# shenyunhang/DRN-WSOD-pytorch

Hardware: AMD Instinct MI355X
Metric: images/sec training, VOC07 DRN-WSOD R50-C4 2k proposals, 1/2/4/8 GPUs (higher is better)
Workload: dtype bf16

## Files before the change

drn-wsod-pytorch_amd/csrc/gemm_conv.hip:

```cpp
#include "drn_common.h"
#include "tune.h"
#include "conv_params.h"

#include <limits.h>

namespace {

struct GemmParams {
  const char* A;
  const char* B;
  float* C;
  int M, N, K;
  long lda, ldb, ldc;
  int k_slabs_per_split;
  long c_split_stride;
  int accumulate;
  float* sgd_w;
  float* sgd_mom;
  bf16_t* sgd_shadow;
  const SgdSeg* sgd_seg;
  float sgd_momentum, sgd_grad_scale;
  int sgd_first_step;
  long sgd_ld;
  int c_bf16;
  int nsplit;
  int gm;
  int kb_rows;
  const float* sgd_acc;
  long sgd_acc_ld;
};

using drn_conv::ConvParams;

template <int DT>
__device__ __forceinline__ void mma_step(f32x16_t& acc, const i32x4_t& a, const i32x4_t& b) {
  if constexpr (DT == DRN_BF16) {
    acc = __builtin_amdgcn_mfma_f32_32x32x16_bf16(__builtin_bit_cast(bf16x8_t, a), __builtin_bit_cast(bf16x8_t, b),
                                                  acc, 0, 0, 0);
  } else if constexpr (DT == DRN_FP8) {
    typedef long i64x2_t __attribute__((ext_vector_type(2)));
    const i64x2_t al = __builtin_bit_cast(i64x2_t, a), bl = __builtin_bit_cast(i64x2_t, b);
    acc = __builtin_amdgcn_mfma_f32_32x32x16_fp8_fp8(al[0], bl[0], acc, 0, 0, 0);
    acc = __builtin_amdgcn_mfma_f32_32x32x16_fp8_fp8(al[1], bl[1], acc, 0, 0, 0);
  } else {
    const f32x4_t af = __builtin_bit_cast(f32x4_t, a), bf = __builtin_bit_cast(f32x4_t, b);
#pragma unroll
    for (int e = 0; e < 4; ++e) acc = __builtin_amdgcn_mfma_f32_32x32x2f32(af[e], bf[e], acc, 0, 0, 0);
  }
}

typedef int i32x8_t __attribute__((ext_vector_type(8)));
__device__ __forceinline__ void mma_step64_fp8(f32x16_t& acc, const i32x4_t& a0, const i32x4_t& a1, const i32x4_t& b0,
                                               const i32x4_t& b1) {
  const i32x8_t A = {a0[0], a0[1], a0[2], a0[3], a1[0], a1[1], a1[2], a1[3]};
  const i32x8_t B = {b0[0], b0[1], b0[2], b0[3], b1[0], b1[1], b1[2], b1[3]};
  acc = __builtin_amdgcn_mfma_scale_f32_32x32x64_f8f6f4(A, B, acc, 0, 0, 0, 0x7f7f7f7f, 0, 0x7f7f7f7f);
}

template <int ROWS>
__device__ __forceinline__ void lds_store_tile(char* lds, const i32x4_t (&r)[ROWS / 32], int tid) {
  const int slot = tid & 7, r0 = tid >> 3;
#pragma unroll
// ... 258 lines not shown
  float lr, wd, mom, gs;
  int first;
};
typedef float f32x2_t_ __attribute__((ext_vector_type(2)));
struct SgdRegs { f32x4_t w, m; f32x2_t_ g; };

__device__ __forceinline__ void sgdp_load(const SgdPipe& sp, SgdRegs& r, unsigned off, unsigned goff) {
  r.w = __builtin_nontemporal_load((const f32x4_t*)((const char*)sp.w + off));
  r.m = __builtin_nontemporal_load((const f32x4_t*)((const char*)sp.m + off));
  r.g = __builtin_nontemporal_load((const f32x2_t_*)((const char*)sp.g + goff));
}
__device__ __forceinline__ void sgdp_apply_store(const SgdPipe& sp, const SgdRegs& r, unsigned off) {
#pragma clang fp contract(off)
  typedef unsigned u32x2_t __attribute__((ext_vector_type(2)));
  const u32x2_t x = __builtin_bit_cast(u32x2_t, r.g);
  const f32x4_t gg = {__builtin_bit_cast(float, x.x << 16), __builtin_bit_cast(float, x.x & 0xffff0000u),
                      __builtin_bit_cast(float, x.y << 16), __builtin_bit_cast(float, x.y & 0xffff0000u)};
  f32x4_t nb, nw;
#pragma unroll
  for (int e = 0; e < 4; ++e) {
    float d = gg[e] * sp.gs;
    if (sp.wd != 0.f) d = d + sp.wd * r.w[e];
    nb[e] = sp.first ? d : sp.mom * r.m[e] + d;
    nw[e] = r.w[e] - sp.lr * nb[e];
  }
  u32x2_t o;
  o.x = (uint32_t)f32_to_bf16(nw[0]) | ((uint32_t)f32_to_bf16(nw[1]) << 16);
  o.y = (uint32_t)f32_to_bf16(nw[2]) | ((uint32_t)f32_to_bf16(nw[3]) << 16);
  __builtin_nontemporal_store(nb, (f32x4_t*)((char*)sp.m + off));
  __builtin_nontemporal_store(nw, (f32x4_t*)((char*)sp.w + off));
  *(u32x2_t*)((char*)sp.s + (off >> 1)) = o;
}

template <int DT, int VAR, bool TN = false, bool SGDP = false>
__device__ __forceinline__ void pp_mainloop(f32x16_t (&acc)[4][2], char* smem, __amdgpu_buffer_rsrc_t ra,
                                            __amdgpu_buffer_rsrc_t rb, const unsigned (&voa)[4], const unsigned (&vob)[4],
                                            int s0, int s1, int lane, int wave, unsigned bstep = 128,
                                            const SgdPipe* spp = nullptr) {
  SgdRegs srA, srB;
  const int wm = wave >> 2, wn = wave & 3;
  const int l31 = lane & 31, hi = lane >> 5, sw = (l31 >> 1) & 7;
  unsigned oa[4], ob[4];
  const unsigned lds0 = (unsigned)(uintptr_t)(__attribute__((address_space(3))) char*)smem;
#pragma unroll
  for (int ks = 0; ks < 4; ++ks) {
    oa[ks] = lds0 + PP_A0 + (wm * 64 + l31) * 128 + (((ks * 2 + hi) ^ sw) << 4);
    const int tg = lane >> 4, tj = (lane >> 2) & 3, tc = lane & 3;
    ob[ks] = TN ? lds0 + PP_B0 + (ks * 4 + 2 * (tg >> 1)) * 1024 + tj * 256 + (((wn * 2 + (tg & 1)) ^ (2 * tj)) << 5) + tc * 8
                : lds0 + PP_B0 + (wn * 32 + l31) * 128 + (((ks * 2 + hi) ^ sw) << 4);
  }
  typedef __attribute__((address_space(3))) const i32x4_t* lds_v4;
  i32x4_t fa[2][4], fb[4];
  auto rdA = [&](int ks, int off) {
    fa[0][ks] = *(lds_v4)(uintptr_t)(oa[ks] + off);
    fa[1][ks] = *(lds_v4)(uintptr_t)(oa[ks] + off + 4096);
  };
  auto rdB = [&](int ks, int off) {
    if constexpr (TN) {
      typedef int i32x2_t __attribute__((ext_vector_type(2)));
      i32x2_t l2, h2;
      const unsigned addr = ob[ks] + off;
      asm volatile("ds_read_b64_tr_b16 %0, %1" : "=v"(l2) : "v"(addr));
      asm volatile("ds_read_b64_tr_b16 %0, %1 offset:1024" : "=v"(h2) : "v"(addr));
      fb[ks] = i32x4_t{l2[0], l2[1], h2[0], h2[1]};
    } else {
      fb[ks] = *(lds_v4)(uintptr_t)(ob[ks] + off);
    }
  };
  auto mm = [&](f32x16_t& c0, f32x16_t& c1, auto wait_b_tag) {
    constexpr bool WAIT_B = decltype(wait_b_tag)::value;
    if (VAR != 3) __builtin_amdgcn_s_setprio(1);
    if constexpr (TN && WAIT_B) asm volatile("s_waitcnt lgkmcnt(6)" : "+v"(fb[0]));
    mma_step<DT>(c0, fb[0], fa[0][0]);
    mma_step<DT>(c1, fb[0], fa[1][0]);
    if constexpr (TN && WAIT_B) { __builtin_amdgcn_sched_barrier(0); asm volatile("s_waitcnt lgkmcnt(4)" : "+v"(fb[1])); }
    mma_step<DT>(c0, fb[1], fa[0][1]);
    mma_step<DT>(c1, fb[1], fa[1][1]);
    if constexpr (TN && WAIT_B) { __builtin_amdgcn_sched_barrier(0); asm volatile("s_waitcnt lgkmcnt(2)" : "+v"(fb[2])); }
    mma_step<DT>(c0, fb[2], fa[0][2]);
    mma_step<DT>(c1, fb[2], fa[1][2]);
    if constexpr (TN && WAIT_B) { __builtin_amdgcn_sched_barrier(0); asm volatile("s_waitcnt lgkmcnt(0)" : "+v"(fb[3])); }
    mma_step<DT>(c0, fb[3], fa[0][3]);
    mma_step<DT>(c1, fb[3], fa[1][3]);
    if (VAR != 3) __builtin_amdgcn_s_setprio(0);
  };
  constexpr std::false_type NOWAIT{};
  constexpr std::true_type WAITB{};
  auto piece = [&](char* stage, auto qtag, int slab) {
    constexpr int q = decltype(qtag)::value;
    constexpr int which = q >> 1, pc = q & 1;
    constexpr int off = which == 0 ? PP_A0 : which == 1 ? PP_B0 : which == 2 ? PP_B1 : PP_A1;
    constexpr bool isA = which == 0 || which == 3;
    constexpr int h = (which == 2 || which == 3) ? 1 : 0;
    char* dst = stage + off + (pc * 64 + wave * 8) * 128;
    __builtin_amdgcn_raw_ptr_buffer_load_lds(isA ? ra : rb, (__attribute__((address_space(3))) void*)dst, 16,
                                             isA ? voa[h * 2 + pc] : vob[h * 2 + pc], isA ? slab * 128 : slab * bstep, 0, 0);
  };
#define PP_PIECE(q) piece(nxt, std::integral_constant<int, q>{}, sn)
  asm volatile("s_waitcnt vmcnt(0)" ::: "memory");
  PP_BARRIER();
  if (wm == 1) PP_BARRIER();
  auto slab = [&](int s, SgdRegs& sr_ld, const SgdRegs& sr_use) __attribute__((always_inline)) {
    char* nxt = smem + (((s - s0) & 1) ^ 1) * PP_STAGE;
    const int sn = s + 1 < s1 ? s + 1 : s1 - 1;
    if constexpr (TN) {
#pragma unroll
      for (int ks = 0; ks < 4; ++ks) rdB(ks, 0);
#pragma unroll
      for (int ks = 0; ks < 4; ++ks) rdA(ks, 0);
    } else {
#pragma unroll
      for (int ks = 0; ks < 4; ++ks) { rdB(ks, 0); rdA(ks, 0); }
    }
    if (VAR == 2) {
      asm volatile("s_waitcnt vmcnt(2)" ::: "memory");
    } else {
      PP_PIECE(0); PP_PIECE(1);
      if constexpr (SGDP) {
        const unsigned i_ = (unsigned)(s - s0);
        if (i_ < 32) {
          sgdp_load(*spp, sr_ld, spp->off + i_ * spp->step, spp->goff + i_ * spp->gstep);
          asm volatile("s_waitcnt vmcnt(7)" ::: "memory");
        } else {
          asm volatile("s_waitcnt vmcnt(4)" ::: "memory");
        }
      } else {
        asm volatile("s_waitcnt vmcnt(4)" ::: "memory");
      }
    }
    PP_BARRIER();
    mm(acc[0][0], acc[1][0], NOWAIT);
    PP_BARRIER();
#pragma unroll
    for (int ks = 0; ks < 4; ++ks) rdB(ks, PP_B1 - PP_B0);
    if (VAR == 2) {
      PP_PIECE(0); PP_PIECE(1); PP_PIECE(2);
      asm volatile("s_waitcnt vmcnt(3)" ::: "memory");
    } else {
      PP_PIECE(2); PP_PIECE(3);
      if constexpr (SGDP) {
        if ((unsigned)(s - s0) < 32) asm volatile("s_waitcnt vmcnt(7)" ::: "memory");
        else asm volatile("s_waitcnt vmcnt(4)" ::: "memory");
      } else asm volatile("s_waitcnt vmcnt(4)" ::: "memory");
    }
    PP_BARRIER();
    mm(acc[0][1], acc[1][1], WAITB);
    PP_BARRIER();
#pragma unroll
    for (int ks = 0; ks < 4; ++ks) rdA(ks, PP_A1 - PP_A0);
    if (VAR == 2) { PP_PIECE(3); PP_PIECE(4); } else { PP_PIECE(4); PP_PIECE(5); }
    if constexpr (SGDP) {
      const unsigned i_ = (unsigned)(s - s0);
      if (i_ >= 1 && i_ <= 32) sgdp_apply_store(*spp, sr_use, spp->off + (i_ - 1) * spp->step);
    }
    PP_BARRIER();
    mm(acc[2][1], acc[3][1], NOWAIT);
    PP_BARRIER();
#pragma unroll
    for (int ks = 0; ks < 4; ++ks) rdB(ks, 0);
    if (VAR == 2) { PP_PIECE(5); PP_PIECE(6); PP_PIECE(7); } else { PP_PIECE(6); PP_PIECE(7); }
    if constexpr (SGDP) {
      if (s > s0 && s - s0 <= 32) asm volatile("s_waitcnt vmcnt(7)" ::: "memory");
      else asm volatile("s_waitcnt vmcnt(4)" ::: "memory");
    } else
    asm volatile("s_waitcnt vmcnt(4)" ::: "memory");
    PP_BARRIER();
    mm(acc[2][0], acc[3][0], WAITB);
    PP_BARRIER();
#pragma unroll
    for (int ks = 0; ks < 4; ++ks) { oa[ks] ^= PP_STAGE; ob[ks] ^= PP_STAGE; }
  };
  if constexpr (SGDP) {
    int s = s0;
    for (; s + 1 < s1; s += 2) {
      slab(s, srA, srB);
      slab(s + 1, srB, srA);
    }
    if (s < s1) slab(s, srA, srB);
  } else {
    for (int s = s0; s < s1; ++s) slab(s, srA, srA);
  }
  asm volatile("s_waitcnt vmcnt(0)" ::: "memory");
  if constexpr (SGDP) {
    const unsigned S = (unsigned)(s1 - s0);
    if (S <= 32) {
      if (S & 1) sgdp_apply_store(*spp, srA, spp->off + (S - 1) * spp->step);
      else sgdp_apply_store(*spp, srB, spp->off + (S - 1) * spp->step);
    }
    for (unsigned c = S; c < 32; c += 4) {
      SgdRegs q[4];
#pragma unroll
      for (unsigned j = 0; j < 4; ++j) {
        const unsigned cc = c + j < 32 ? c + j : 31;
        sgdp_load(*spp, q[j], spp->off + cc * spp->step, spp->goff + cc * spp->gstep);
      }
#pragma unroll
      for (unsigned j = 0; j < 4; ++j)
        if (c + j < 32) sgdp_apply_store(*spp, q[j], spp->off + (c + j) * spp->step);
    }
  }
// ... 181 lines not shown
          *(f32x4_t*)dst = v;
        } else {
#pragma unroll
          for (int e = 0; e < 4; ++e)
            if (n + e < p.N) dst[e] = p.accumulate ? dst[e] + v[e] : v[e];
        }
      }
  }
}

struct GemmWork { int bm, bn, s0, s1, split; __amdgpu_buffer_rsrc_t ra, rb; };

template <int DT, int PP = 0, bool TN = false, bool PAIR = false, bool SGDP = false, bool ACC = false>
__global__ __launch_bounds__(512) void gemm_nt256p_kernel(GemmParams p_in, GemmParams p2_in, int pair_wg0) {
  extern __shared__ __attribute__((aligned(16))) char smem[];
  const bool second = PAIR && (int)(blockIdx.x >> 3) >= pair_wg0;
  const GemmParams p = second ? p2_in : p_in;
  constexpr int ES = DT == DRN_BF16 ? 2 : 4;
  constexpr int BM = 256, BN = 256, MI = 4, NJ = 2;
  constexpr int A_BYTES = BM * 128, STAGE = (BM + BN) * 128;
  const int tiles_m = (p.M + BM - 1) / BM, tiles_n = (p.N + BN - 1) / BN;
  const int tiles = tiles_m * tiles_n;
  const int total = tiles * p.nsplit;
  const int nslab = p.K * ES / 128;
  const int tid = threadIdx.x, lane = tid & 63;
  const int wave = __builtin_amdgcn_readfirstlane(tid >> 6);
  const int wm = wave >> 2, wn = wave & 3;
  const int bid = blockIdx.x;
  const int per = PAIR ? (second ? (int)(gridDim.x >> 3) - pair_wg0 : pair_wg0) : (int)(gridDim.x >> 3);
  const int xcd = bid & 7, q = total >> 3, r = total & 7;
  const int base = xcd < r ? xcd * (q + 1) : r * (q + 1) + (xcd - r) * q;
  const int len = q + (xcd < r ? 1 : 0);
  int j = PAIR ? (second ? (bid >> 3) - pair_wg0 : (bid >> 3)) : (bid >> 3);
  if (j >= len) return;
  const unsigned lda_b = (unsigned)(p.lda * ES), ldb_b = (unsigned)(p.ldb * ES);
  unsigned voa[4], vob[4];
#pragma unroll
  for (int i = 0; i < 4; ++i) {
    const unsigned row = i * 64 + (tid >> 3), ks = (tid & 7) ^ ((row >> 1) & 7);
    voa[i] = row * lda_b + ks * 16;
    vob[i] = row * ldb_b + ks * 16;
  }
  using Work = GemmWork;
  auto setup = [&](int logical, Work& w) {
    w.split = logical / tiles;
    int tm, tn;
    tile_coords(logical - w.split * tiles, tiles_m, tiles_n, tm, tn, p.gm);
    w.bm = tm * BM;
    w.bn = tn * BN;
    w.s0 = w.split * p.k_slabs_per_split;
    w.s1 = w.s0 + p.k_slabs_per_split < nslab ? w.s0 + p.k_slabs_per_split : nslab;
    w.ra = make_row_loader(p.A, w.bm, p.M, BM, p.lda * ES).rsrc;
    w.rb = TN ? make_tn_rsrc(p.B, w.bn, p.kb_rows, p.ldb * ES, ES) : make_row_loader(p.B, w.bn, p.N, BN, p.ldb * ES).rsrc;
  };
  const unsigned bstep = TN ? 64u * ldb_b : 128u;
  auto issue = [&](const Work& w, char* stage, int slab) {
#pragma unroll
    for (int i = 0; i < 4; ++i) {
      char* dst = stage + (i * 64 + wave * 8) * 128;
      __builtin_amdgcn_raw_ptr_buffer_load_lds(w.ra, (__attribute__((address_space(3))) void*)dst, 16, voa[i], slab * 128, 0, 0);
      __builtin_amdgcn_raw_ptr_buffer_load_lds(w.rb, (__attribute__((address_space(3))) void*)(dst + A_BYTES), 16, vob[i], slab * 128, 0, 0);
    }
  };
  f32x16_t acc[MI][NJ];
  auto load_frags = [&](const char* buf, int ks, i32x4_t (&fa)[MI], i32x4_t (&fb)[NJ]) {
    const int slot = ks * 2 + (lane >> 5);
#pragma unroll
    for (int i = 0; i < MI; ++i) fa[i] = *(const i32x4_t*)(buf + swz(wm * 128 + i * 32 + (lane & 31), slot));
#pragma unroll
    for (int jj = 0; jj < NJ; ++jj) fb[jj] = *(const i32x4_t*)(buf + A_BYTES + swz(wn * 64 + jj * 32 + (lane & 31), slot));
  };
  auto mma_all = [&](const i32x4_t (&fa)[MI], const i32x4_t (&fb)[NJ]) {
#pragma unroll
    for (int i = 0; i < MI; ++i)
#pragma unroll
      for (int jj = 0; jj < NJ; ++jj) mma_step<DT>(acc[i][jj], fb[jj], fa[i]);
  };
  unsigned pva[4], pvb[4];
  if constexpr (PP) pp_offsets<TN>(lda_b, ldb_b, tid, pva, pvb);
  Work cur;
  setup(base + j, cur);
  if (cur.s0 < cur.s1) {
    if constexpr (PP) pp_issue_first(smem, cur.ra, cur.rb, pva, pvb, wave, cur.s0, bstep);
    else issue(cur, smem, cur.s0);
  }
  [[maybe_unused]] SgdPipe sp;
  [[maybe_unused]] bool have_prev = false;
  if constexpr (SGDP) {
    sp.w = p.sgd_w; sp.m = p.sgd_mom; sp.g = (const bf16_t*)p.C; sp.s = p.sgd_shadow;
    sp.step = (unsigned)(8 * p.sgd_ld * 4); sp.gstep = (unsigned)(8 * p.ldc * 2);
    sp.lr = p.sgd_seg->lr; sp.wd = p.sgd_seg->wd; sp.mom = p.sgd_momentum; sp.gs = p.sgd_grad_scale;
    sp.first = p.sgd_first_step;
    sp.off = sp.goff = 0;
  }
  for (;;) {
#pragma unroll
    for (int i = 0; i < MI; ++i)
#pragma unroll
      for (int jj = 0; jj < NJ; ++jj)
#pragma unroll
        for (int rr = 0; rr < 16; ++rr) acc[i][jj][rr] = 0.f;
    const int s0 = cur.s0, s1 = cur.s1;
    if constexpr (PP) {
      if constexpr (SGDP) {
        if (have_prev) pp_mainloop<DT, PP, TN, true>(acc, smem, cur.ra, cur.rb, pva, pvb, s0, s1, lane, wave, bstep, &sp);
        else pp_mainloop<DT, PP, TN>(acc, smem, cur.ra, cur.rb, pva, pvb, s0, s1, lane, wave, bstep);
      } else if (s0 < s1) pp_mainloop<DT, PP, TN>(acc, smem, cur.ra, cur.rb, pva, pvb, s0, s1, lane, wave, bstep);
    } else if (s0 < s1) {
      i32x4_t fa0[MI], fb0[NJ], fa1[MI], fb1[NJ];
      asm volatile("s_waitcnt vmcnt(0)" ::: "memory");
      __builtin_amdgcn_s_barrier();
      if (s0 + 1 < s1) issue(cur, smem + STAGE, s0 + 1);
      load_frags(smem, 0, fa0, fb0);
#define DRN_INTERLEAVE()                                                     \
  _Pragma("unroll") for (int q_ = 0; q_ < 6; ++q_) {                           \
    __builtin_amdgcn_sched_group_barrier(0x008, 1, 0);                        \
    __builtin_amdgcn_sched_group_barrier(0x100, 1, 0);                        \
  }                                                                          \
  __builtin_amdgcn_sched_group_barrier(0x008, 2, 0)
      int s = s0;
      for (; s + 1 < s1; ++s) {
        char* cs = smem + ((s - s0) & 1) * STAGE;
        char* nx = smem + (((s - s0) & 1) ^ 1) * STAGE;
        load_frags(cs, 1, fa1, fb1);
        mma_all(fa0, fb0);
        DRN_INTERLEAVE();
        load_frags(cs, 2, fa0, fb0);
        mma_all(fa1, fb1);
        DRN_INTERLEAVE();
        load_frags(cs, 3, fa1, fb1);
        mma_all(fa0, fb0);
        DRN_INTERLEAVE();
        asm volatile("s_waitcnt vmcnt(0) lgkmcnt(0)" ::: "memory");
        __builtin_amdgcn_s_barrier();
        issue(cur, cs, s + 2 < s1 ? s + 2 : s1 - 1);
        load_frags(nx, 0, fa0, fb0);
        mma_all(fa1, fb1);
#pragma unroll
        for (int q_ = 0; q_ < 6; ++q_) {
          __builtin_amdgcn_sched_group_barrier(0x008, 1, 0);
          __builtin_amdgcn_sched_group_barrier(0x100, 1, 0);
          __builtin_amdgcn_sched_group_barrier(0x020, 1, 0);
        }
        __builtin_amdgcn_sched_group_barrier(0x008, 1, 0);
        __builtin_amdgcn_sched_group_barrier(0x020, 1, 0);
        __builtin_amdgcn_sched_group_barrier(0x008, 1, 0);
        __builtin_amdgcn_sched_group_barrier(0x020, 1, 0);
      }
      {
        char* cs = smem + ((s - s0) & 1) * STAGE;
        load_frags(cs, 1, fa1, fb1);
        mma_all(fa0, fb0);
        DRN_INTERLEAVE();
        load_frags(cs, 2, fa0, fb0);
        mma_all(fa1, fb1);
        DRN_INTERLEAVE();
        load_frags(cs, 3, fa1, fb1);
        mma_all(fa0, fb0);
        DRN_INTERLEAVE();
        mma_all(fa1, fb1);
        asm volatile("s_waitcnt vmcnt(0)" ::: "memory");
      }
#undef DRN_INTERLEAVE
    }
    j += per;
    const bool more = j < len;
    Work nxt;
    if (more) {
      setup(base + j, nxt);
      asm volatile("s_waitcnt lgkmcnt(0)" ::: "memory");
      __builtin_amdgcn_s_barrier();
      if (nxt.s0 < nxt.s1) {
        if constexpr (PP) pp_issue_first(smem, nxt.ra, nxt.rb, pva, pvb, wave, nxt.s0, bstep);
        else issue(nxt, smem, nxt.s0);
      }
    }
    const int bm = cur.bm, bn = cur.bn;
    if (p.c_bf16 && (p.ldc & 7) == 0 && (((uintptr_t)p.C) & 15) == 0) {
      const unsigned ep = (unsigned)(uintptr_t)(__attribute__((address_space(3))) char*)(smem + STAGE);
      bf16_t* C16 = (bf16_t*)p.C;
      int lane_e = lane, tid_e = tid;
      asm volatile("" : "+v"(lane_e), "+v"(tid_e));
      if (!more) { asm volatile("s_waitcnt lgkmcnt(0)" ::: "memory"); __builtin_amdgcn_s_barrier(); }
      if constexpr (ACC) {
        static_assert(TN && SGDP, "the accumulating epilogue belongs to the fused TN dW + SGD launch (whole tiles)");
        const float* ga = p.sgd_acc + (long)(bm + wm * 128 + (lane_e & 31)) * p.sgd_acc_ld + bn + wn * 32 + 4 * (lane_e >> 5);
#pragma unroll
        for (int i = 0; i < MI; ++i) {
          const float* gi = ga + (long)(i * 32) * p.sgd_acc_ld;
          f32x4_t o[NJ][4];
#pragma unroll
          for (int jj = 0; jj < NJ; ++jj)
#pragma unroll
            for (int qq = 0; qq < 4; ++qq) o[jj][qq] = __builtin_nontemporal_load((const f32x4_t*)(gi + jj * 128 + 8 * qq));
#pragma unroll
          for (int jj = 0; jj < NJ; ++jj)
#pragma unroll
            for (int qq = 0; qq < 4; ++qq)
#pragma unroll
              for (int e = 0; e < 4; ++e) acc[i][jj][4 * qq + e] = acc[i][jj][4 * qq + e] + o[jj][qq][e];
        }
      }
#pragma unroll
      for (int half = 0; half < 2; ++half) {
        if (wm == half) {
#pragma unroll
          for (int i = 0; i < MI; ++i) {
            const int row = i * 32 + (lane_e & 31);
#pragma unroll
            for (int jj = 0; jj < NJ; ++jj)
#pragma unroll
              for (int qq = 0; qq < 4; ++qq) {
                const int c = (TN ? jj * 32 + wn * 8 : wn * 16 + jj * 8) + 2 * qq + (lane_e >> 5);
                const unsigned long long o =
                    (unsigned long long)((uint32_t)f32_to_bf16(acc[i][jj][4 * qq]) | ((uint32_t)f32_to_bf16(acc[i][jj][4 * qq + 1]) << 16)) |
                    ((unsigned long long)((uint32_t)f32_to_bf16(acc[i][jj][4 * qq + 2]) | ((uint32_t)f32_to_bf16(acc[i][jj][4 * qq + 3]) << 16)) << 32);
                asm volatile("ds_write_b64 %0, %1" ::"v"(ep + row * 512 + ((c ^ ((row & 31) << 1)) << 3)), "v"(o) : "memory");
              }
            __builtin_amdgcn_sched_barrier(0);
          }
        }
        asm volatile("s_waitcnt lgkmcnt(0)" ::: "memory");
        __builtin_amdgcn_s_barrier();
        if (SGDP && (p.c_bf16 & 2)) {
#pragma unroll 1
          for (int it = 0; it < 8; it += 4) {
            i32x4_t v0, v1, v2, v3;
            const int r0_ = (it * 512 + tid_e) >> 5, pc_ = tid_e & 31;
            asm volatile("ds_read_b128 %0, %4\n\tds_read_b128 %1, %5\n\tds_read_b128 %2, %6\n\tds_read_b128 %3, %7\n\ts_waitcnt lgkmcnt(0)"
                         : "=&v"(v0), "=&v"(v1), "=&v"(v2), "=&v"(v3)
                         : "v"(ep + (r0_) * 512 + ((pc_ ^ ((r0_) & 31)) << 4)), "v"(ep + (r0_ + 16) * 512 + ((pc_ ^ ((r0_ + 16) & 31)) << 4)),
                           "v"(ep + (r0_ + 32) * 512 + ((pc_ ^ ((r0_ + 32) & 31)) << 4)), "v"(ep + (r0_ + 48) * 512 + ((pc_ ^ ((r0_ + 48) & 31)) << 4))
                         : "memory");
            bf16_t* dst = C16 + (long)(bm + half * 128 + r0_) * p.ldc + bn + pc_ * 8;
            *(i32x4_t*)dst = v0;
            *(i32x4_t*)(dst + 16 * p.ldc) = v1;
            *(i32x4_t*)(dst + 32 * p.ldc) = v2;
            *(i32x4_t*)(dst + 48 * p.ldc) = v3;
          }
        } else
#pragma unroll 1
        for (int it = 0; it < 8; ++it) {
          const int idx = it * 512 + tid_e;
          const int row = idx >> 5, pc = idx & 31;
          const int m = bm + half * 128 + row, n = bn + pc * 8;
          i32x4_t v;
          asm volatile("ds_read_b128 %0, %1\n\ts_waitcnt lgkmcnt(0)" : "=v"(v) : "v"(ep + row * 512 + ((pc ^ (row & 31)) << 4)) : "memory");
          if (m < p.M) {
            bf16_t* dst = C16 + (long)m * p.ldc + n;
            if (n + 8 <= p.N) {
              *(i32x4_t*)dst = v;
            } else {
              const bf16_t* e8 = (const bf16_t*)&v;
#pragma unroll
              for (int e = 0; e < 8; ++e)
                if (n + e < p.N) dst[e] = e8[e];
            }
// ... 15 lines not shown
            const int n = bn + (TN ? jj * 128 + wn * 32 : wn * 64 + jj * 32) + 8 * qq + 4 * (lane >> 5);
            float* dst = C + (long)m * p.ldc + n;
            f32x4_t v = {acc[i][jj][4 * qq], acc[i][jj][4 * qq + 1], acc[i][jj][4 * qq + 2], acc[i][jj][4 * qq + 3]};
            if (p.c_bf16) {
              bf16_t* d16 = (bf16_t*)p.C + (long)m * p.ldc + n;
              if (vec_ok && n + 4 <= p.N) {
                uint2 o;
                o.x = (uint32_t)f32_to_bf16(v[0]) | ((uint32_t)f32_to_bf16(v[1]) << 16);
                o.y = (uint32_t)f32_to_bf16(v[2]) | ((uint32_t)f32_to_bf16(v[3]) << 16);
                *(uint2*)d16 = o;
              } else {
#pragma unroll
                for (int e = 0; e < 4; ++e)
                  if (n + e < p.N) d16[e] = f32_to_bf16(v[e]);
              }
            } else if (vec_ok && n + 4 <= p.N) {
              if (p.accumulate) { const f32x4_t o = *(const f32x4_t*)dst; v += o; }
              *(f32x4_t*)dst = v;
            } else {
#pragma unroll
              for (int e = 0; e < 4; ++e)
                if (n + e < p.N) dst[e] = p.accumulate ? dst[e] + v[e] : v[e];
            }
          }
      }
    }
    if constexpr (SGDP) {
      sp.off = (unsigned)(((long)(bm + wave) * p.sgd_ld + bn + lane * 4) * 4);
      sp.goff = (unsigned)(((long)(bm + wave) * p.ldc + bn + lane * 4) * 2);
      have_prev = true;
    }
    if (!more) break;
    cur = nxt;
  }
  if constexpr (SGDP) {
    asm volatile("s_waitcnt vmcnt(0)" ::: "memory");
    __builtin_amdgcn_s_barrier();
    for (unsigned c = 0; c < 32; c += 2) {
      SgdRegs q0, q1;
      sgdp_load(sp, q0, sp.off + c * sp.step, sp.goff + c * sp.gstep);
      sgdp_load(sp, q1, sp.off + (c + 1) * sp.step, sp.goff + (c + 1) * sp.gstep);
      sgdp_apply_store(sp, q0, sp.off + c * sp.step);
      sgdp_apply_store(sp, q1, sp.off + (c + 1) * sp.step);
    }
  }
}

__global__ __launch_bounds__(512) void conv1x1_pp_kernel(ConvParams p) {
  extern __shared__ __attribute__((aligned(16))) char smem[];
  const int Mtot = p.Nb * p.Ho * p.Wo;
  const int tiles_m = (Mtot + 255) / 256, tiles_n = (p.Cout + 255) / 256;
  int tm, tn;
  tile_coords(xcd_remap(blockIdx.x, tiles_m * tiles_n), tiles_m, tiles_n, tm, tn, 4);
  const int bm = tm * 256, bn = tn * 256;
  const int tid = threadIdx.x, lane = tid & 63;
  const int wave = __builtin_amdgcn_readfirstlane(tid >> 6);
  const int wm = wave >> 2, wn = wave & 3;
  const RowLoader la = make_row_loader(p.X, bm, Mtot, 256, (long)p.Cin * 2);
  const RowLoader lb = make_row_loader(p.Wt, bn, p.Cout, 256, p.ldw * 2);
  unsigned pva[4], pvb[4];
  pp_offsets<false>(la.ld_bytes, lb.ld_bytes, tid, pva, pvb);
  f32x16_t acc[4][2];
#pragma unroll
  for (int i = 0; i < 4; ++i)
#pragma unroll
    for (int j = 0; j < 2; ++j)
#pragma unroll
      for (int r = 0; r < 16; ++r) acc[i][j][r] = 0.f;
  const int nslab = p.Cin >> 6;
  pp_issue_first(smem, la.rsrc, lb.rsrc, pva, pvb, wave, 0);
// ... 843 lines not shown
       return old;
     }},
    {10, &DrnTune::roi_cpb, [](int v, int cur) { return v >= 1 && v <= 64 && (v & (v - 1)) == 0 ? v : cur; }},
    {11, &DrnTune::roi_prefetch, tune_truthy},
    {12, &DrnTune::gemm_pingpong, [](int v, int) { return v < 0 ? 0 : v; }},
    {13, &DrnTune::fp8_k64, tune_truthy},
    {14, &DrnTune::roi_map64_a, tune_truthy},
    {15, &DrnTune::roi_lds_kb, tune_range<60, 154>},
    {18, &DrnTune::gemm_nwg, [](int v, int cur) { return v >= 0 && v % 8 == 0 && v <= 4096 ? v : cur; }},
    {19, nullptr, [](int v, int) {
       const int old = g_tune.roi_lane;
       g_tune.roi_walk_nsg = v == 3 ? 1 : 2;
       g_tune.roi_lane = v < 0 ? 0 : v == 3 ? 1 : v > 2 ? 2 : v;
       return old;
     }},
    {20, &DrnTune::sgdp_ep4, tune_truthy},
    {22, &DrnTune::roi_lane_reps, tune_range<0, 64>},
    {23, &DrnTune::conv_ring, tune_one_of<0, 1, 64, 128>},
    {24, &DrnTune::conv_pp, tune_range<0, INT_MAX>},
    {25, &DrnTune::pp8, tune_range<0, 2>},
    {26, &DrnTune::pp8_stages, tune_one_of<3, 4, 5>},
    {27, &DrnTune::pp8_var, [](int v, int cur) { return v >= 0 && v <= 10 && (v & 3) != 3 ? v : cur; }},
    {28, nullptr, [](int, int) { return drn_tune_pp8_profile_dump(); }},
    {29, &DrnTune::pp8_wide, tune_range<0, 2>},
    {30, &DrnTune::pp8_wvar, tune_one_of<0, 1, 4, 5, 8, 9, 13>},
    {31, nullptr, [](int v, int) {
       const int old = g_tune.roi_st;
       g_tune.roi_st = tune_range<0, 2>(v, old);
       if (v == 10 || v == 11) g_tune.roi_st_prof = v == 10;
       if (v == 12 && drn_tune_roi_st_profile_dump() != 0) return -1;
       return old;
     }},
    {32, &DrnTune::msm_wave, tune_truthy},
};
}

static int gemm_tn_sgd_entry(const void* A, const void* Bt, void* grad_bucket, const float* grad_acc, long ld_acc, int M, int N,
                             int K, int kb_rows, long lda, long ldb, long ldc, float* weights, float* momentum_buf, void* shadow,
                             long ld_w, const void* seg_dev, float momentum, int first_step, float grad_scale, void* stream) {
  if (!A || !Bt || !grad_bucket || !weights || !momentum_buf || !seg_dev || M <= 0 || N <= 0 || K <= 0 || kb_rows < 0 ||
      kb_rows > K)
    return DRN_ERR_ARG;
  if (lda < K || ldb < N || ldc < N || ld_w < N) return DRN_ERR_ARG;
  if ((lda * 2) % 16 != 0 || (ldb * 2) % 16 != 0 ||
      (((uintptr_t)A | (uintptr_t)Bt | (uintptr_t)grad_bucket | (uintptr_t)weights | (uintptr_t)momentum_buf | (uintptr_t)shadow) & 15))
    return DRN_ERR_UNSUPPORTED;
  if (K < 128 || (K & 63) || (M & 255) || (N & 255) || !shadow || (ldc & 7) || (ld_w & 3) || g_tune.gemm_pingpong != 1 ||
      (long)M * ld_w * 4 >= 0xFFFFFFF0L || (long)K * ldb * 2 >= 0xFFFFFFF0L)
    return DRN_ERR_UNSUPPORTED;
  if (grad_acc && ((ld_acc & 3) || (((uintptr_t)grad_acc) & 15) || (long)M * ld_acc * 4 >= 0xFFFFFFF0L)) return DRN_ERR_UNSUPPORTED;
  const long tiles = (long)(M / 256) * (N / 256);
  const int nwg = persistent_grid(tiles);
  if (!nwg) return DRN_ERR_UNSUPPORTED;
  GemmParams p{(const char*)A, (const char*)Bt, (float*)grad_bucket, M, N, K, lda, ldb, ldc, K * 2 / 128, 0, 0,
               weights, momentum_buf, (bf16_t*)shadow, (const SgdSeg*)seg_dev, momentum, grad_scale, first_step};
  p.sgd_ld = ld_w;
  p.c_bf16 = g_tune.sgdp_ep4 ? 3 : 1;
  p.nsplit = 1;
  p.gm = gemm256_group_rows(M, N, 1);
  p.kb_rows = kb_rows;
  if (grad_acc) {
    p.sgd_acc = grad_acc;
    p.sgd_acc_ld = ld_acc;
    return launch_gemm256p_tn_acc_sgdp(p, nwg, (hipStream_t)stream);
  }
  return launch_gemm256p_tn_sgdp(p, nwg, (hipStream_t)stream);
}

extern "C" {

int drn_gemm_set_tile(int tile) {
  const int old = g_tune.force_tile;
  if (tile == 0 || tile == 64 || tile == 128 || tile == 255 || tile == 256) g_tune.force_tile = tile;
  return old;
}

int drn_tune(int knob, int value) {
  for (const TuneRow& row : kTuneRows) {
    if (row.id != knob) continue;
    if (!row.field) return row.accept(value, 0);
    const int old = g_tune.*row.field;
    g_tune.*row.field = row.accept(value, old);
    return old;
  }
  return -1;
}

long drn_gemm_nt_main_cols(int M, int N, int splits) {
  if (M <= 0 || N <= 0 || splits < 1) return N;
  const long wg256 = (long)((M + 255) / 256) * ((N + 255) / 256) * splits;
  if (!((g_tune.force_tile == 256 || (g_tune.force_tile == 0 && wg256 >= 192)))) return N;
  const int nwg = persistent_grid(wg256);
  return nwg ? tail_split_main_cols(M, N, splits, nwg) : N;
// ... 227 lines not shown
```

drn-wsod-pytorch_amd/csrc/tune.h:

```cpp
#pragma once

struct DrnTune {
  int gemm_persistent = 1;
  int sgd_grid = 512;
  int gemm_group_rows = 0;
  int roi_map64 = 512;
  int conv_ksplit = 1;
  int gemm_tail_split = 1;
  int conv_ks_tiles = 0;
  int conv_k2_tiles = -1;
  int conv_patch = 1;
  int conv_patch_min = 32768;
  int roi_cpb = 1;
  int roi_prefetch = 1;
  int gemm_pingpong = 1;
  int fp8_k64 = 1;
  int roi_map64_a = 0;
  int roi_lds_kb = 154;
  int gemm_nwg = 0;
  int roi_lane = 1;
  int roi_walk_nsg = 2;
  int sgdp_ep4 = 1;
  int roi_lane_reps = 0;
  int conv_ring = 1;
  int conv_pp = 1;
  int pp8 = 1;
  int pp8_stages = 5;
  int pp8_var = 1;
  int pp8_wide = 1;
  int pp8_wvar = 4;
  int roi_st = 1;
  int roi_st_prof = 0;
  int msm_wave = 1;
  int force_tile = 0;
};

extern __attribute__((visibility("hidden"))) DrnTune g_tune;

__attribute__((visibility("hidden"))) int drn_tune_pp8_profile_dump();
__attribute__((visibility("hidden"))) int drn_tune_roi_st_profile_dump();
```

drn-wsod-pytorch_amd/ops.py:

```python
import contextlib
import ctypes
import functools
import math

import torch

from . import _cabi as C

SCALE_CLAMP = math.log(1000.0 / 16)
GEMM_TIMING = None
HBM_TIMING = None


FP8 = torch.float8_e4m3fn
FP8_MAX = 448.0


def esize(dtype):
    return 1 if dtype == FP8 else 2 if dtype == torch.bfloat16 else 4


def kpad(k, dtype):
    q = 128 // esize(dtype)
    return (k + q - 1) // q * q
# ... 7 lines not shown
def gemm_set_tile(tile):
    return C.lib().drn_gemm_set_tile(int(tile))


TUNE_GEMM_PERSISTENT = 1
TUNE_SGD_GRID = 2
TUNE_GEMM_GROUP_ROWS = 3
TUNE_ROI_MAP64 = 4
TUNE_CONV_KSPLIT = 5
TUNE_GEMM_TAIL_SPLIT = 6
TUNE_CONV_KS_TILES = 7
TUNE_CONV_K2_TILES = 8
TUNE_CONV_PATCH = 9
TUNE_ROI_CPB = 10
TUNE_ROI_PREFETCH = 11
TUNE_GEMM_PINGPONG = 12
TUNE_FP8_K64 = 13
TUNE_ROI_MAP64_A = 14
TUNE_ROI_LDS_KB = 15
TUNE_GEMM_NWG = 18
TUNE_ROI_LANE = 19
TUNE_SGDP_EPILOGUE = 20
TUNE_ROI_LANE_REPS = 22
TUNE_CONV_RING = 23
TUNE_CONV_PP = 24
TUNE_PP8 = 25
TUNE_PP8_STAGES = 26
TUNE_PP8_VARIANT = 27
TUNE_PP8_PROFILE = 28
TUNE_PP8_WIDE = 29
TUNE_PP8_WIDE_VARIANT = 30
TUNE_ROI_ST = 31
TUNE_MSM_WAVE = 32


def tune(knob, value):
    return C.lib().drn_tune(int(knob), int(value))


@contextlib.contextmanager
def tuned(knobs=None, tile=None):
    prev, undo = {}, []
    try:
        if tile is not None:
            prev["tile"] = gemm_set_tile(tile)
            undo.append((gemm_set_tile, prev["tile"]))
        for k, v in (knobs or {}).items():
            prev[k] = tune(k, v)
            undo.append((functools.partial(tune, k), prev[k]))
        yield prev
    finally:
        for fn, old in reversed(undo):
            fn(old)


def gemm_nt(A, B, M, N, K, out=None, splits=1, accumulate=False):
    lda, ldb = _2d(A), _2d(B)
    assert A.dtype == B.dtype
    if out is None:
        out = torch.empty((splits, M, N), dtype=torch.float32, device=A.device)
    assert out.dtype == torch.float32 or (out.dtype == torch.bfloat16 and splits == 1 and not accumulate)
    ldc = out.stride(-2)
    sstride = out.stride(0) if out.dim() == 3 else 0
    assert out.dim() == 3 or splits == 1
    if GEMM_TIMING is not None:
        e0, e1 = torch.cuda.Event(enable_timing=True), torch.cuda.Event(enable_timing=True)
# ... 701 lines not shown
```

include/drn_wsod.h:

```cpp
#ifndef DRN_WSOD_H_
#define DRN_WSOD_H_
#include <stdint.h>

#ifdef __cplusplus
extern "C" {
#endif

#define DRN_OK 0
#define DRN_ERR_ARG (-1)
#define DRN_ERR_LAUNCH (-2)
#define DRN_ERR_UNSUPPORTED (-3)
#define DRN_F32 0
#define DRN_BF16 1


int drn_preprocess_nhwc(const float* img_chw, int C, int H, int W, void* out_nhwc, int Hp, int Wp, int Cp,
                        const float* mean3_host, const float* std3_host, int dtype, void* stream);

int drn_resize_bilinear_u8(const void* src_hwc, int H, int W, int C, float* dst_chw, int Ho, int Wo, const int* xbounds,
                           const int* xcoef, int ksx, const int* ybounds, const int* ycoef, int ksy, int flip, void* stream);

int drn_conv2d_nhwc(const void* x, const void* w, void* y, const float* scale, const float* bias,
                    const void* residual, int Nb, int H, int W, int Cin, int Cout, int KH, int KW, int stride,
                    int pad, int dil, long ldw, long ldy, long ldres, int relu, int dtype, void* stream);
// ... 87 lines not shown
                        const void* seg_dev, float momentum, int first_step, float grad_scale, void* stream);

int drn_gemm_set_tile(int tile);

#define DRN_TUNE_GEMM_PERSISTENT 1
#define DRN_TUNE_SGD_GRID 2
#define DRN_TUNE_GEMM_GROUP_ROWS 3
#define DRN_TUNE_ROI_MAP64 4
#define DRN_TUNE_CONV_KSPLIT 5
#define DRN_TUNE_GEMM_TAIL_SPLIT 6
#define DRN_TUNE_CONV_KS_TILES 7
#define DRN_TUNE_CONV_K2_TILES 8
#define DRN_TUNE_CONV_PATCH 9
#define DRN_TUNE_ROI_CPB 10
#define DRN_TUNE_ROI_PREFETCH 11
#define DRN_TUNE_GEMM_PINGPONG 12
#define DRN_TUNE_FP8_K64 13
#define DRN_TUNE_ROI_MAP64_A 14
#define DRN_TUNE_ROI_LDS_KB 15
#define DRN_TUNE_GEMM_NWG 18
#define DRN_TUNE_ROI_LANE 19
#define DRN_TUNE_SGDP_EPILOGUE 20
#define DRN_TUNE_ROI_LANE_REPS 22
#define DRN_TUNE_CONV_RING 23
#define DRN_TUNE_CONV_PP 24
#define DRN_TUNE_PP8 25
#define DRN_TUNE_PP8_STAGES 26
#define DRN_TUNE_PP8_VARIANT 27
#define DRN_TUNE_PP8_PROFILE 28
#define DRN_TUNE_PP8_WIDE 29
#define DRN_TUNE_PP8_WIDE_VARIANT 30
#define DRN_TUNE_ROI_ST 31
#define DRN_TUNE_MSM_WAVE 32
int drn_tune(int knob, int value);

int drn_linear_act_fwd(const void* A, const void* W, const float* bias, const float* mask, unsigned long long seed,
                       const unsigned long long* seed_dev, float drop_p, void* out, long ld_out, void* outT, long ld_outT,
                       int M, int N, int K, long lda, long ldw, int relu, void* stream);

int drn_bias_act_fwd(const float* partials, int splits, long split_stride, const float* bias, const float* mask,
                     unsigned long long seed, const unsigned long long* seed_dev, float drop_p, void* out, long ld_out,
                     void* outT, long ld_outT, int M, int N, long ld_in, int relu, int out_dtype, void* stream);

int drn_counter_add(unsigned long long* counter, unsigned long long inc, void* stream);

int drn_bias_act_bwd(const void* grad_out, int grad_dtype, long ld_in, const float* colscale, const int* colidx,
                     const void* saved_out, const float* mask, float drop_p,
                     void* dpre, long ld_out, void* dpreT, long ld_outT, float* colsum, float* colpart,
                     int accumulate_colsum, int M, int N, int out_dtype, void* stream);

int drn_bias_act_bwd_splits(const void* grad_out, int grad_dtype, long ld_in, int splits, long split_stride,
                            const float* colscale, const int* colidx, const void* saved_out, const float* mask,
                            float drop_p, void* dpre, long ld_out, void* dpreT, long ld_outT, float* colsum,
                            float* colpart, int accumulate_colsum, int M, int N, int out_dtype, void* stream);

int drn_gemm_nt_act_bwd(const void* A, const void* B, int M, int N, int K, long lda, long ldb, const void* saved_out,
                        const float* mask, float drop_p, void* dpre, long ld_out, void* dpreT, long ld_outT, float* colsum,
                        float* colpart, int accumulate_colsum, void* stream);

int drn_colsum_reduce(const float* colpart, int nparts, int N, float* colsum, int accumulate, void* stream);


int drn_wsddn_fwd_bwd(const float* logits, long ld, int c_cls, int c_det, int K, const int* img_off, int n_img,
                      const float* gt_onehot, float* scores, float* row_softmax, float* img_scores, float* loss_part,
                      float* dlogits, long ld_d, float* scratch, int max_rows, int mean_loss, float loss_scale,
                      void* stream);
// ... 110 lines not shown
```

Measured before the change: 797.6.

## Split tail tiles of fused SGD GEMM into sub-tile pieces across idle workgroups

```diff
diff --git a/drn-wsod-pytorch_amd/csrc/gemm_conv.hip b/drn-wsod-pytorch_amd/csrc/gemm_conv.hip
--- a/drn-wsod-pytorch_amd/csrc/gemm_conv.hip
+++ b/drn-wsod-pytorch_amd/csrc/gemm_conv.hip
@@ -28,6 +28,7 @@
   int kb_rows;
   const float* sgd_acc;
   long sgd_acc_ld;
+  int sgd_tail;
 };
 
 using drn_conv::ConvParams;
@@ -352,11 +353,14 @@
   *(u32x2_t*)((char*)sp.s + (off >> 1)) = o;
 }
 
-template <int DT, int VAR, bool TN = false, bool SGDP = false>
+template <int DT, int VAR, bool TN = false, bool SGDP = false, bool PIECE = false>
 __device__ __forceinline__ void pp_mainloop(f32x16_t (&acc)[4][2], char* smem, __amdgpu_buffer_rsrc_t ra,
                                             __amdgpu_buffer_rsrc_t rb, const unsigned (&voa)[4], const unsigned (&vob)[4],
                                             int s0, int s1, int lane, int wave, unsigned bstep = 128,
-                                            const SgdPipe* spp = nullptr) {
+                                            const SgdPipe* spp = nullptr, unsigned imask = 15, unsigned jmask = 3) {
+  [[maybe_unused]] const bool qa0 = !PIECE || (imask & 3), qa1 = !PIECE || (imask & 12);
+  [[maybe_unused]] const bool qb0 = !PIECE || (jmask & 1), qb1 = !PIECE || (jmask & 2);
+  [[maybe_unused]] const bool e0 = !PIECE || (imask & 5), e1 = !PIECE || (imask & 10);
   SgdRegs srA, srB;
   const int wm = wave >> 2, wn = wave & 3;
   const int l31 = lane & 31, hi = lane >> 5, sw = (l31 >> 1) & 7;
@@ -387,21 +391,24 @@
       fb[ks] = *(lds_v4)(uintptr_t)(ob[ks] + off);
     }
   };
-  auto mm = [&](f32x16_t& c0, f32x16_t& c1, auto wait_b_tag) {
+  auto mm = [&](f32x16_t& c0, f32x16_t& c1, auto wait_b_tag, [[maybe_unused]] bool on = true) {
     constexpr bool WAIT_B = decltype(wait_b_tag)::value;
+    if constexpr (PIECE) {
+      if (!on) return;
+    }
     if (VAR != 3) __builtin_amdgcn_s_setprio(1);
     if constexpr (TN && WAIT_B) asm volatile("s_waitcnt lgkmcnt(6)" : "+v"(fb[0]));
-    mma_step<DT>(c0, fb[0], fa[0][0]);
-    mma_step<DT>(c1, fb[0], fa[1][0]);
+    if (!PIECE || e0) mma_step<DT>(c0, fb[0], fa[0][0]);
+    if (!PIECE || e1) mma_step<DT>(c1, fb[0], fa[1][0]);
     if constexpr (TN && WAIT_B) { __builtin_amdgcn_sched_barrier(0); asm volatile("s_waitcnt lgkmcnt(4)" : "+v"(fb[1])); }
-    mma_step<DT>(c0, fb[1], fa[0][1]);
-    mma_step<DT>(c1, fb[1], fa[1][1]);
+    if (!PIECE || e0) mma_step<DT>(c0, fb[1], fa[0][1]);
+    if (!PIECE || e1) mma_step<DT>(c1, fb[1], fa[1][1]);
     if constexpr (TN && WAIT_B) { __builtin_amdgcn_sched_barrier(0); asm volatile("s_waitcnt lgkmcnt(2)" : "+v"(fb[2])); }
-    mma_step<DT>(c0, fb[2], fa[0][2]);
-    mma_step<DT>(c1, fb[2], fa[1][2]);
+    if (!PIECE || e0) mma_step<DT>(c0, fb[2], fa[0][2]);
+    if (!PIECE || e1) mma_step<DT>(c1, fb[2], fa[1][2]);
     if constexpr (TN && WAIT_B) { __builtin_amdgcn_sched_barrier(0); asm volatile("s_waitcnt lgkmcnt(0)" : "+v"(fb[3])); }
-    mma_step<DT>(c0, fb[3], fa[0][3]);
-    mma_step<DT>(c1, fb[3], fa[1][3]);
+    if (!PIECE || e0) mma_step<DT>(c0, fb[3], fa[0][3]);
+    if (!PIECE || e1) mma_step<DT>(c1, fb[3], fa[1][3]);
     if (VAR != 3) __builtin_amdgcn_s_setprio(0);
   };
   constexpr std::false_type NOWAIT{};
@@ -423,7 +430,17 @@
   auto slab = [&](int s, SgdRegs& sr_ld, const SgdRegs& sr_use) __attribute__((always_inline)) {
     char* nxt = smem + (((s - s0) & 1) ^ 1) * PP_STAGE;
     const int sn = s + 1 < s1 ? s + 1 : s1 - 1;
-    if constexpr (TN) {
+    if constexpr (PIECE) {
+      static_assert(!PIECE || TN, "tail pieces: the TN form only");
+      if (qa0 && qb0) {
+#pragma unroll
+        for (int ks = 0; ks < 4; ++ks) rdB(ks, 0);
+      }
+      if (qa0) {
+#pragma unroll
+        for (int ks = 0; ks < 4; ++ks) rdA(ks, 0);
+      }
+    } else if constexpr (TN) {
 #pragma unroll
       for (int ks = 0; ks < 4; ++ks) rdB(ks, 0);
 #pragma unroll
@@ -449,10 +466,12 @@
       }
     }
     PP_BARRIER();
-    mm(acc[0][0], acc[1][0], NOWAIT);
+    mm(acc[0][0], acc[1][0], NOWAIT, qa0 && qb0);
     PP_BARRIER();
-#pragma unroll
-    for (int ks = 0; ks < 4; ++ks) rdB(ks, PP_B1 - PP_B0);
+    if (!PIECE || qb1) {
+#pragma unroll
+      for (int ks = 0; ks < 4; ++ks) rdB(ks, PP_B1 - PP_B0);
+    }
     if (VAR == 2) {
       PP_PIECE(0); PP_PIECE(1); PP_PIECE(2);
       asm volatile("s_waitcnt vmcnt(3)" ::: "memory");
@@ -464,20 +483,24 @@
       } else asm volatile("s_waitcnt vmcnt(4)" ::: "memory");
     }
     PP_BARRIER();
-    mm(acc[0][1], acc[1][1], WAITB);
+    mm(acc[0][1], acc[1][1], WAITB, qa0 && qb1);
     PP_BARRIER();
-#pragma unroll
-    for (int ks = 0; ks < 4; ++ks) rdA(ks, PP_A1 - PP_A0);
+    if (!PIECE || qa1) {
+#pragma unroll
+      for (int ks = 0; ks < 4; ++ks) rdA(ks, PP_A1 - PP_A0);
+    }
     if (VAR == 2) { PP_PIECE(3); PP_PIECE(4); } else { PP_PIECE(4); PP_PIECE(5); }
     if constexpr (SGDP) {
       const unsigned i_ = (unsigned)(s - s0);
       if (i_ >= 1 && i_ <= 32) sgdp_apply_store(*spp, sr_use, spp->off + (i_ - 1) * spp->step);
     }
     PP_BARRIER();
-    mm(acc[2][1], acc[3][1], NOWAIT);
+    mm(acc[2][1], acc[3][1], NOWAIT, qa1 && qb1);
     PP_BARRIER();
-#pragma unroll
-    for (int ks = 0; ks < 4; ++ks) rdB(ks, 0);
+    if (!PIECE || (qa1 && qb0)) {
+#pragma unroll
+      for (int ks = 0; ks < 4; ++ks) rdB(ks, 0);
+    }
     if (VAR == 2) { PP_PIECE(5); PP_PIECE(6); PP_PIECE(7); } else { PP_PIECE(6); PP_PIECE(7); }
     if constexpr (SGDP) {
       if (s > s0 && s - s0 <= 32) asm volatile("s_waitcnt vmcnt(7)" ::: "memory");
@@ -485,7 +508,7 @@
     } else
     asm volatile("s_waitcnt vmcnt(4)" ::: "memory");
     PP_BARRIER();
-    mm(acc[2][0], acc[3][0], WAITB);
+    mm(acc[2][0], acc[3][0], WAITB, qa1 && qb0);
     PP_BARRIER();
 #pragma unroll
     for (int ks = 0; ks < 4; ++ks) { oa[ks] ^= PP_STAGE; ob[ks] ^= PP_STAGE; }
@@ -733,6 +756,17 @@
   const int base = xcd < r ? xcd * (q + 1) : r * (q + 1) + (xcd - r) * q;
   const int len = q + (xcd < r ? 1 : 0);
   int j = PAIR ? (second ? (bid >> 3) - pair_wg0 : (bid >> 3)) : (bid >> 3);
+  [[maybe_unused]] int tp_n = 0, tp_rem = 0;
+  if constexpr (SGDP) {
+    const int rm = len % per;
+    if (p.sgd_tail && rm && 2 * rm <= per && len > per) {
+      int n = 8 * rm <= per ? 8 : 4 * rm <= per ? 4 : 2;
+      if (p.sgd_tail > 1 && p.sgd_tail < n) n = p.sgd_tail;
+      tp_n = n;
+      tp_rem = rm;
+    }
+  }
+  [[maybe_unused]] const int full = len - tp_rem, j0 = j;
   if (j >= len) return;
   const unsigned lda_b = (unsigned)(p.lda * ES), ldb_b = (unsigned)(p.ldb * ES);
   unsigned voa[4], vob[4];
@@ -779,6 +813,25 @@
   };
   unsigned pva[4], pvb[4];
   if constexpr (PP) pp_offsets<TN>(lda_b, ldb_b, tid, pva, pvb);
+  [[maybe_unused]] unsigned imask = 15, jmask = 3;
+  [[maybe_unused]] bool cur_piece = false;
+  [[maybe_unused]] auto piece_setup = [&]() {
+    const int pi = j0 % tp_n;
+    if (tp_n == 2) { imask = 3u << (2 * pi); jmask = 3; }
+    else if (tp_n == 4) { imask = 3u << (2 * (pi >> 1)); jmask = 1u << (pi & 1); }
+    else { imask = 1u << (pi >> 1); jmask = 1u << (pi & 1); }
+    const unsigned span_a = (unsigned)nslab * 128u, span_b = (unsigned)nslab * bstep;
+    int tid_p = tid;
+    asm volatile("" : "+v"(tid_p));
+    const bool fit_a = 256ul * lda_b + span_a < 0x7FFFFFF0ul, fit_b = (unsigned long)nslab * bstep < 0x7FFFFFF0ul;
+#pragma unroll
+    for (int h = 0; h < 2; ++h)
+#pragma unroll
+      for (int pc = 0; pc < 2; ++pc) {
+        if (fit_a && !((imask >> (2 * h + (tid_p >> 8))) & 1)) pva[h * 2 + pc] = 0xFFFFFFF0u - span_a;
+        if (fit_b && !((jmask >> h) & 1)) pvb[h * 2 + pc] = 0xFFFFFFF0u - span_b;
+      }
+  };
   Work cur;
   setup(base + j, cur);
   if (cur.s0 < cur.s1) {
@@ -804,7 +857,9 @@
     const int s0 = cur.s0, s1 = cur.s1;
     if constexpr (PP) {
       if constexpr (SGDP) {
-        if (have_prev) pp_mainloop<DT, PP, TN, true>(acc, smem, cur.ra, cur.rb, pva, pvb, s0, s1, lane, wave, bstep, &sp);
+        if (cur_piece)
+          pp_mainloop<DT, PP, TN, true, true>(acc, smem, cur.ra, cur.rb, pva, pvb, s0, s1, lane, wave, bstep, &sp, imask, jmask);
+        else if (have_prev) pp_mainloop<DT, PP, TN, true>(acc, smem, cur.ra, cur.rb, pva, pvb, s0, s1, lane, wave, bstep, &sp);
         else pp_mainloop<DT, PP, TN>(acc, smem, cur.ra, cur.rb, pva, pvb, s0, s1, lane, wave, bstep);
       } else if (s0 < s1) pp_mainloop<DT, PP, TN>(acc, smem, cur.ra, cur.rb, pva, pvb, s0, s1, lane, wave, bstep);
     } else if (s0 < s1) {
@@ -865,10 +920,19 @@
 #undef DRN_INTERLEAVE
     }
     j += per;
-    const bool more = j < len;
+    bool more = j < len;
+    [[maybe_unused]] bool nxt_piece = false;
+    if constexpr (SGDP) {
+      more = j < full;
+      if (!more && !cur_piece && j0 < tp_rem * tp_n) {
+        more = nxt_piece = true;
+        piece_setup();
+      }
+    }
     Work nxt;
     if (more) {
-      setup(base + j, nxt);
+      if constexpr (SGDP) setup(nxt_piece ? base + full + j0 / tp_n : base + j, nxt);
+      else setup(base + j, nxt);
       asm volatile("s_waitcnt lgkmcnt(0)" ::: "memory");
       __builtin_amdgcn_s_barrier();
       if (nxt.s0 < nxt.s1) {
@@ -877,7 +941,7 @@
       }
     }
     const int bm = cur.bm, bn = cur.bn;
-    if (p.c_bf16 && (p.ldc & 7) == 0 && (((uintptr_t)p.C) & 15) == 0) {
+    if (SGDP || (p.c_bf16 && (p.ldc & 7) == 0 && (((uintptr_t)p.C) & 15) == 0)) {
       const unsigned ep = (unsigned)(uintptr_t)(__attribute__((address_space(3))) char*)(smem + STAGE);
       bf16_t* C16 = (bf16_t*)p.C;
       int lane_e = lane, tid_e = tid;
@@ -888,6 +952,7 @@
         const float* ga = p.sgd_acc + (long)(bm + wm * 128 + (lane_e & 31)) * p.sgd_acc_ld + bn + wn * 32 + 4 * (lane_e >> 5);
 #pragma unroll
         for (int i = 0; i < MI; ++i) {
+          if (cur_piece && !((imask >> i) & 1)) continue;
           const float* gi = ga + (long)(i * 32) * p.sgd_acc_ld;
           f32x4_t o[NJ][4];
 #pragma unroll
@@ -923,7 +988,20 @@
         }
         asm volatile("s_waitcnt lgkmcnt(0)" ::: "memory");
         __builtin_amdgcn_s_barrier();
-        if (SGDP && (p.c_bf16 & 2)) {
+        bool piece_ep = false;
+        if constexpr (SGDP) piece_ep = cur_piece;
+        if (piece_ep) {
+#pragma unroll 1
+          for (int it = 0; it < 8; ++it) {
+            const int idx = it * 512 + tid_e;
+            const int row = idx >> 5, pc = idx & 31;
+            if (((imask >> (row >> 5)) & 1) && ((jmask >> (pc >> 4)) & 1)) {
+              i32x4_t v;
+              asm volatile("ds_read_b128 %0, %1\n\ts_waitcnt lgkmcnt(0)" : "=v"(v) : "v"(ep + row * 512 + ((pc ^ (row & 31)) << 4)) : "memory");
+              *(i32x4_t*)(C16 + (long)(bm + half * 128 + row) * p.ldc + bn + pc * 8) = v;
+            }
+          }
+        } else if (SGDP && (p.c_bf16 & 2)) {
 #pragma unroll 1
           for (int it = 0; it < 8; it += 4) {
             i32x4_t v0, v1, v2, v3;
@@ -1005,10 +1083,31 @@
     }
     if (!more) break;
     cur = nxt;
+    if constexpr (SGDP) cur_piece = nxt_piece;
   }
   if constexpr (SGDP) {
     asm volatile("s_waitcnt vmcnt(0)" ::: "memory");
     __builtin_amdgcn_s_barrier();
+    if (cur_piece) {
+      const bool halfc = jmask != 3;
+      int lane_d = lane;
+      asm volatile("" : "+v"(lane_d));
+      const unsigned lr = halfc ? wave + (lane_d >> 5) : 0;
+      const int dcol = halfc ? (int)(jmask >> 1) * 128 + (lane_d & 31) * 4 - lane_d * 4 : 0;
+      const unsigned nch = halfc ? 2 : 4, cstep = halfc ? 2 : 1;
+      const unsigned o0 = sp.off + lr * (sp.step >> 3) + dcol * 4, g0 = sp.goff + lr * (sp.gstep >> 3) + dcol * 2;
+      for (unsigned b = 0; b < 8; ++b) {
+        if (!((imask >> (b & 3)) & 1)) continue;
+        for (unsigned c = 0; c < nch; c += 2) {
+          const unsigned c0 = b * 4 + c * cstep, c1 = c0 + cstep;
+          SgdRegs q0, q1;
+          sgdp_load(sp, q0, o0 + c0 * sp.step, g0 + c0 * sp.gstep);
+          sgdp_load(sp, q1, o0 + c1 * sp.step, g0 + c1 * sp.gstep);
+          sgdp_apply_store(sp, q0, o0 + c0 * sp.step);
+          sgdp_apply_store(sp, q1, o0 + c1 * sp.step);
+        }
+      }
+    } else
     for (unsigned c = 0; c < 32; c += 2) {
       SgdRegs q0, q1;
       sgdp_load(sp, q0, sp.off + c * sp.step, sp.goff + c * sp.gstep);
@@ -1918,6 +2017,7 @@
        return old;
      }},
     {32, &DrnTune::msm_wave, tune_truthy},
+    {34, &DrnTune::sgdp_tail, tune_one_of<0, 1, 2, 4, 8>},
 };
 }
 
@@ -1945,6 +2045,7 @@
   p.nsplit = 1;
   p.gm = gemm256_group_rows(M, N, 1);
   p.kb_rows = kb_rows;
+  p.sgd_tail = g_tune.sgdp_tail;
   if (grad_acc) {
     p.sgd_acc = grad_acc;
     p.sgd_acc_ld = ld_acc;
diff --git a/drn-wsod-pytorch_amd/csrc/tune.h b/drn-wsod-pytorch_amd/csrc/tune.h
--- a/drn-wsod-pytorch_amd/csrc/tune.h
+++ b/drn-wsod-pytorch_amd/csrc/tune.h
@@ -32,6 +32,7 @@
   int roi_st = 1;
   int roi_st_prof = 0;
   int msm_wave = 1;
+  int sgdp_tail = 1;
   int force_tile = 0;
 };
 
diff --git a/drn-wsod-pytorch_amd/ops.py b/drn-wsod-pytorch_amd/ops.py
--- a/drn-wsod-pytorch_amd/ops.py
+++ b/drn-wsod-pytorch_amd/ops.py
@@ -63,6 +63,7 @@
 TUNE_PP8_WIDE_VARIANT = 30
 TUNE_ROI_ST = 31
 TUNE_MSM_WAVE = 32
+KNOB_SGDP_TAIL_PIECES = 34
 
 
 def tune(knob, value):
diff --git a/include/drn_wsod.h b/include/drn_wsod.h
--- a/include/drn_wsod.h
+++ b/include/drn_wsod.h
@@ -143,6 +143,7 @@
 #define DRN_TUNE_PP8_WIDE_VARIANT 30
 #define DRN_TUNE_ROI_ST 31
 #define DRN_TUNE_MSM_WAVE 32
+enum { DRN_TUNE_SGDP_TAIL_PIECES = 34 };
 int drn_tune(int knob, int value);
 
 int drn_linear_act_fwd(const void* A, const void* W, const float* bias, const float* mask, unsigned long long seed,
```

Measured after the change: 804.9 (median of 6 runs). Within noise of the previous version (+0.9%).
